# ArrowLuo/SegCLIP

Measured on AMD Instinct MI355X. Metric: image-text pairs/s fwd+bwd, ViT-B/16 224^2, per-GPU batch 256 (global 2048 at 8 GPUs), higher is better.
Workload: dtype bf16; 1 GPU; BASELINE configs[1]/[2]: ViT-B/16 224^2 + 77-token text, contrastive loss only; per_gpu_batch=256, global_batch=256, parallelism=dp1, attention_forward=bf16, residual_stream=fp32, cross_mode=t18, text_positions=all 77 (full context, as the reference computes it)

## Files before the change

### segclip_amd/csrc/attention.hip

```cpp
#include <stdlib.h>
#include <algorithm>
#include <atomic>

#include "common.h"

int segclip_gemm_f32_launch(const segclip_gemm_desc* d, hipStream_t stream);

namespace {

typedef __attribute__((address_space(3))) s16x4 lds_s16x4;

constexpr int ROWB = 128;

__device__ __forceinline__ int swz(int row, int col) {
  const int t = (row >> 1) & 7;
  const int f = ((t & 1) << 2) | (t >> 1);
  return row * ROWB + ((((col >> 3) ^ f)) << 4) + ((col & 7) << 1);
}

__device__ __forceinline__ bf16x8_t frag_rows(const char* t, int rbase, int kc, int lane) {
  return *reinterpret_cast<const bf16x8_t*>(t + swz(rbase + (lane & 31), kc * 16 + 8 * (lane >> 5)));
}
__device__ __forceinline__ bf16x8_t frag_tr(const char* t, int rbase, int cbase, int lane) {
  const int g4 = lane >> 4, q = lane & 15;
// ... 445 lines not shown
  stage_rows(Vt, Vp, a.v_st, 0, a.Tk, tkp, a.hd, tid, blockDim.x);
  __syncthreads();

  for (int q0 = wave * 32; q0 < tqp; q0 += nw * 32) {
    bf16x8_t qf[4], gf[4];
#pragma unroll
    for (int kc = 0; kc < 4; ++kc) {
      qf[kc] = frag_rows_g(Qp, a.q_st, q0, a.Tq, kc, lane, a.hd);
      gf[kc] = frag_rows_g(Gp, a.do_st, q0, a.Tq, kc, lane, a.hd);
    }
    const int q = q0 + li;
    const float lq = Ls[q], dq_ = Ds[q];
    f32x16 dq[2];
#pragma unroll
    for (int r = 0; r < 16; ++r) { dq[0][r] = 0.f; dq[1][r] = 0.f; }
    for (int k0 = 0; k0 < tkp; k0 += 32) {
      if (a.causal && k0 > q0 + 31) break;
      f32x16 s, dp;
#pragma unroll
      for (int r = 0; r < 16; ++r) { s[r] = 0.f; dp[r] = 0.f; }
#pragma unroll
      for (int kc = 0; kc < 4; ++kc) {
        s = __builtin_amdgcn_mfma_f32_32x32x16_bf16(frag_rows(Kt, k0, kc, lane), qf[kc], s, 0, 0, 0);
        dp = __builtin_amdgcn_mfma_f32_32x32x16_bf16(frag_rows(Vt, k0, kc, lane), gf[kc], dp, 0, 0, 0);
      }
      const bool edge = k0 + 32 > kvalid || q0 + 32 > a.Tq || (a.causal && k0 + 31 > q0);
      float ds[16];
      if (edge) {
#pragma unroll
        for (int r = 0; r < 16; ++r) {
          const int key = k0 + accrow(r, lh);
          const bool ok = key < kvalid && q < a.Tq && (!a.causal || key <= q);
          ds[r] = ok ? __builtin_amdgcn_exp2f(s[r] * sc2 - lq) * (dp[r] - dq_) : 0.f;
        }
      } else {
#pragma unroll
        for (int r = 0; r < 16; ++r) ds[r] = __builtin_amdgcn_exp2f(s[r] * sc2 - lq) * (dp[r] - dq_);
      }
      const bf16x8_t sb0 = pack8(ds), sb1 = pack8(ds + 8);
#pragma unroll
      for (int dt = 0; dt < 2; ++dt) {
        dq[dt] = __builtin_amdgcn_mfma_f32_32x32x16_bf16(frag_tr(Kt, k0, dt * 32, lane), sb0, dq[dt], 0, 0, 0);
        dq[dt] = __builtin_amdgcn_mfma_f32_32x32x16_bf16(frag_tr(Kt, k0 + 16, dt * 32, lane), sb1, dq[dt], 0, 0, 0);
      }
    }
#pragma unroll
    for (int r = 0; r < 16; ++r) { dq[0][r] *= a.scale; dq[1][r] *= a.scale; }
    store_acc_T(a.dQ + b * a.dq_sb + hoff, a.dq_st, q, a.Tq, a.hd, dq, lh);
  }

  if (a.colsum_part) {
    const int c = tid & 7, nrl = (int)blockDim.x >> 3;
    float accq[8];
#pragma unroll
    for (int j = 0; j < 8; ++j) accq[j] = 0.f;
    for (int r = tid >> 3; r < tkp; r += nrl) {
      const u32x4 kv = *reinterpret_cast<const u32x4*>(Kt + swz(r, c * 8));
      const float w = Cs[r];
#pragma unroll
      for (int j = 0; j < 4; ++j) {
        accq[2 * j] += w * __uint_as_float(kv[j] << 16);
        accq[2 * j + 1] += w * __uint_as_float(kv[j] & 0xffff0000u);
      }
    }
#pragma unroll
    for (int j = 0; j < 8; ++j) {
      float vq = accq[j], vv = accv[j];
      vq += __shfl_xor(vq, 8, 64); vv += __shfl_xor(vv, 8, 64);
      vq += __shfl_xor(vq, 16, 64); vv += __shfl_xor(vv, 16, 64);
      vq += __shfl_xor(vq, 32, 64); vv += __shfl_xor(vv, 32, 64);
      if (lane < 8) {
        Red[(wave * 3 + 0) * 64 + c * 8 + j] = vq;
        Red[(wave * 3 + 2) * 64 + c * 8 + j] = vv;
      }
    }
    __syncthreads();
    for (int t = tid; t < 192; t += (int)blockDim.x) {
      const int m = t >> 6, dd = t & 63;
      float v = 0.f;
      if (m != 1)
        for (int w = 0; w < nw; ++w) v += Red[(w * 3 + m) * 64 + dd];
      if (dd < a.hd) a.colsum_part[((int64_t)b * 3 + m) * ((int64_t)a.H * a.hd) + hoff + dd] = v;
    }
  }
}

#include "attention_sp.inc"
#include "attention_pf.inc"
#include "attention_spl.inc"
#include "attention_dqw.inc"
#include "attention_stream.inc"

__global__ void softmax_rows_kernel(float* __restrict__ S, int64_t rows, int Tq, int Tk, int causal, const int* klen,
                                    int H) {
  const int lane = threadIdx.x & 63;
  const int64_t row = (int64_t)blockIdx.x * (blockDim.x >> 6) + (threadIdx.x >> 6);
  if (row >= rows) return;
  const int q = (int)(row % Tq);
  float* s = S + row * Tk;
  int lim = causal ? (q + 1 < Tk ? q + 1 : Tk) : Tk;
  if (klen) { const int kv = klen[row / ((int64_t)H * Tq)]; lim = kv < lim ? kv : lim; }
  float mx = -INFINITY;
  for (int c = lane; c < lim; c += 64) mx = fmaxf(mx, s[c]);
  mx = wave_max(mx);
  float sum = 0.f;
  for (int c = lane; c < lim; c += 64) sum += expf(s[c] - mx);
  sum = wave_sum(sum);
  const float inv = 1.f / sum;
  for (int c = lane; c < Tk; c += 64) s[c] = c < lim ? expf(s[c] - mx) * inv : 0.f;
}
__global__ void softmax_bwd_rows_kernel(const float* __restrict__ P, float* __restrict__ dP, int64_t rows, int Tk,
                                        float scale) {
  const int lane = threadIdx.x & 63;
  const int64_t row = (int64_t)blockIdx.x * (blockDim.x >> 6) + (threadIdx.x >> 6);
  if (row >= rows) return;
  const float* p = P + row * Tk;
  float* d = dP + row * Tk;
  float dot = 0.f;
  for (int c = lane; c < Tk; c += 64) dot += p[c] * d[c];
  dot = wave_sum(dot);
  for (int c = lane; c < Tk; c += 64) d[c] = p[c] * (d[c] - dot) * scale;
}


bool bf16_ok(const segclip_attn_desc* d) {
  const int64_t s[] = {d->q_sb, d->q_st, d->k_sb, d->k_st, d->v_sb, d->v_st, d->o_sb, d->o_st};
  for (int64_t v : s) if (v % 8) return false;
  return d->hd % 8 == 0 && d->hd <= 64;
}

struct Tuning {
  int smallq = segclip_tuning_int("SEGCLIP_ATTN_SMALLQ", 1);
  int fwd_staged = segclip_tuning_int("SEGCLIP_ATTN_FWD_STAGED", -1), fwd_lean = segclip_tuning_int("SEGCLIP_ATTN_FWD_LEAN", 1);
  int fwd_pf = segclip_tuning_int("SEGCLIP_ATTN_FWD_PF", 1), fwd_grid = segclip_tuning_int("SEGCLIP_ATTN_FWD_GRID", 0);
  int bwd_dqw_long = segclip_tuning_int("SEGCLIP_ATTN_BWD_DQW_LONG", 1), bwd_dqw = segclip_tuning_int("SEGCLIP_ATTN_BWD_DQW", 1);
  int bwd_sp = segclip_tuning_int("SEGCLIP_ATTN_BWD_SP", 1), bwd_spl = segclip_tuning_int("SEGCLIP_ATTN_BWD_SPL", 1);
  int bwd_grid = segclip_tuning_int("SEGCLIP_ATTN_BWD_GRID", -1), bwd_waves = segclip_tuning_int("SEGCLIP_ATTN_BWD_WAVES", 0);
};
const Tuning& tuning() { static const Tuning t; return t; }

struct Plan {
  int route, tiles, variant;
  int waves;
  size_t lds;
  int staged;
};
int tiles_of(const segclip_attn_desc* d) { return (int)cdiv(d->Tq > d->Tk ? d->Tq : d->Tk, 32); }
bool long_seq(const segclip_attn_desc* d) { return d->Tq > TMAX || d->Tk > TMAX; }

Plan plan_fwd(const segclip_attn_desc* d) {
  const Tuning& t = tuning();
  if (d->dtype != SEGCLIP_BF16) return {SEGCLIP_ATTN_ROUTE_F32, tiles_of(d)};
  const int staged = t.fwd_staged >= 0 ? t.fwd_staged : (d->Tq > 128 ? 1 : 0);
  if (t.smallq && smallq::covers(d)) return {SEGCLIP_ATTN_ROUTE_SMALLQ, 1, 0, smallq::WPB_FWD, smallq::lds_bytes((int)d->Tk, false), staged};
  const int tiles = (int)cdiv(d->Tq, 32);
  const size_t pf_lds = fwd_pf_lds_bytes(tiles, (int)d->Tq);
  if (t.fwd_pf && d->Tq == d->Tk && !(d->flags & SEGCLIP_ATTN_FP8) && (tiles == 3 || tiles == 6 || tiles == 7) && pf_lds <= 160 * 1024)
    return {SEGCLIP_ATTN_ROUTE_PF, tiles, d->causal ? 1 : 0, tiles + 1, pf_lds, staged};
  const int nw = tiles < 8 ? tiles : (tiles <= 8 ? 8 : (int)cdiv(tiles, cdiv(tiles, 8)));
  return {SEGCLIP_ATTN_ROUTE_GENERIC, tiles, (staged ? 1 : 0) | nw << 8, nw, 0, staged};
}

Plan plan_bwd(const segclip_attn_desc* d) {
  const Tuning& t = tuning();
  const int tiles = tiles_of(d);
  if (d->dtype != SEGCLIP_BF16) return {SEGCLIP_ATTN_ROUTE_F32, tiles};
  if (t.smallq && smallq::covers(d)) return {SEGCLIP_ATTN_ROUTE_SMALLQ, 1, 0, smallq::WPB_BWD, smallq::lds_bytes((int)d->Tk, true)};
  if (long_seq(d)) {
    if (t.bwd_dqw_long && d->Tq == d->Tk && !d->causal && d->hd == 64 && d->Tq % 32 <= 30 && d->Tq % 224 != 0)
      return {SEGCLIP_ATTN_ROUTE_DQW, 7, 1, 8, bwd_dqw_lds_bytes<7>()};
    return {SEGCLIP_ATTN_ROUTE_STREAM, tiles, 0, 0, bwd_stream_lds_bytes()};
  }
  const bool masked = d->causal || d->klen;
  if (t.bwd_sp && d->Tq == d->Tk) {
    if (t.bwd_dqw && !masked && d->hd == 64 && tiles == 7 && d->Tq % 32 >= 1 && d->Tq % 32 <= 30)
      return {SEGCLIP_ATTN_ROUTE_DQW, 7, 0, 8, bwd_dqw_lds_bytes<7>()};
    const size_t spl_lds = bwd_spl_lds_bytes((int)d->Tq);
    if (t.bwd_spl && !masked && d->hd == 64 && tiles >= 5 && tiles <= 7 && spl_lds <= 160 * 1024)
      return {SEGCLIP_ATTN_ROUTE_SPL, tiles, 0, tiles + 1, spl_lds};
    return {SEGCLIP_ATTN_ROUTE_SP, tiles, masked ? 1 : 0, tiles, bwd_sp_lds_bytes(tiles * 32)};
  }
  int nw = tiles < 4 ? tiles : 4;
  if (t.bwd_waves >= 1 && t.bwd_waves <= 8) nw = tiles < t.bwd_waves ? tiles : t.bwd_waves;
  return {SEGCLIP_ATTN_ROUTE_TWOPASS, tiles, nw << 8, nw, bwd_lds_bytes(tiles * 32)};
}

constexpr int MAX_DEVICES = 64;
struct Device { int index, ncu; };
std::atomic<int> device_ncu[MAX_DEVICES];
std::atomic<int> pf_per_cu[MAX_DEVICES][2][8][33];

bool current_device(Device& dv) {
  if (hipGetDevice(&dv.index) != hipSuccess || dv.index < 0 || dv.index >= MAX_DEVICES) return false;
  if ((dv.ncu = device_ncu[dv.index]) == 0) {
    if (hipDeviceGetAttribute(&dv.ncu, hipDeviceAttributeMultiprocessorCount, dv.index) != hipSuccess || dv.ncu <= 0) dv.ncu = 256;
    device_ncu[dv.index] = dv.ncu;
  }
  return true;
}

template <auto KERNEL>
int raise_lds_limit(const char* who, const Device& dv, size_t bytes) {
  static std::atomic<bool> done[MAX_DEVICES];
  if (done[dv.index]) return 0;
  const hipError_t e = hipFuncSetAttribute(reinterpret_cast<const void*>(KERNEL), hipFuncAttributeMaxDynamicSharedMemorySize, (int)bytes);
  SEGCLIP_REQUIRE(e == hipSuccess, "%s bf16: cannot raise the dynamic LDS limit: %s", who, hipGetErrorString(e));
  done[dv.index] = true;
  return 0;
}

template <auto KERNEL, typename... Args>
int launch(const char* name, dim3 grid, int waves, const Plan& p, hipStream_t stream, const Args&... args) {
  hipLaunchKernelGGL(KERNEL, grid, dim3(waves * 64), p.lds, stream, args...);
  SEGCLIP_CHECK_LAUNCH(name);
  return 0;
}

template <int NT, bool CAUSAL>
int launch_fwd_pf_as(const FwdArgs& a, const Plan& p, int nitems, hipStream_t stream) {
  Device dv;
  SEGCLIP_REQUIRE(current_device(dv), "attn_fwd: cannot query the current device");
  if (int rc = raise_lds_limit<attn_fwd_pf_kernel<NT, CAUSAL>>("attn_fwd", dv, 160 * 1024)) return rc;
  std::atomic<int>& cached = pf_per_cu[dv.index][CAUSAL][NT][pf_kv_rows(a.Tq) >> 3];
  int per_cu = cached;
  if (per_cu == 0) {
    if (hipOccupancyMaxActiveBlocksPerMultiprocessor(&per_cu, attn_fwd_pf_kernel<NT, CAUSAL>, p.waves * 64, p.lds) != hipSuccess || per_cu < 1) per_cu = 1;
    if (tuning().fwd_grid > 0) per_cu = tuning().fwd_grid;
    cached = per_cu;
  }
  return launch<attn_fwd_pf_kernel<NT, CAUSAL>>("attn_fwd_pf", dim3(std::min(nitems, dv.ncu * per_cu)), p.waves, p, stream, a, nitems);
}
int launch_fwd_pf(const FwdArgs& a, const Plan& p, int nitems, hipStream_t stream) {
  switch (p.tiles * 2 + p.variant) {
    case 3 * 2: return launch_fwd_pf_as<3, false>(a, p, nitems, stream);
    case 3 * 2 + 1: return launch_fwd_pf_as<3, true>(a, p, nitems, stream);
    case 6 * 2: return launch_fwd_pf_as<6, false>(a, p, nitems, stream);
    case 6 * 2 + 1: return launch_fwd_pf_as<6, true>(a, p, nitems, stream);
    case 7 * 2: return launch_fwd_pf_as<7, false>(a, p, nitems, stream);
    default: return launch_fwd_pf_as<7, true>(a, p, nitems, stream);
  }
}

int launch_fwd_generic(const segclip_attn_desc* d, const FwdArgs& a, const Plan& p, hipStream_t stream) {
  SEGCLIP_REQUIRE(d->B * d->H <= 65535, "attn_fwd: B*H too large");
  if (d->flags & SEGCLIP_ATTN_FP8) {
    segclip_set_error("attn_fwd: the e4m3 forward was removed (slower than bf16 at head_dim 64, DESIGN.md section 8): "
                      "configs[4] runs bf16 attention");
    return SEGCLIP_ERR_UNSUPPORTED;
  }
  return launch<attn_fwd_bf16_kernel>("attn_fwd_bf16", dim3((unsigned)cdiv(p.tiles, p.waves), (unsigned)(d->B * d->H)), p.waves, p, stream, a);
}

struct Mat { const void* p; int64_t s0, sk, sb, sh; };
int gemm_f32(const segclip_attn_desc* d, hipStream_t stream, int64_t M, int64_t N, int64_t K, Mat A, Mat B, Mat C, float alpha = 1.f) {
  segclip_gemm_desc g{};
  g.nb1 = d->B; g.nb2 = d->H;
  g.a_dtype = g.b_dtype = g.c_dtype = g.r_dtype = SEGCLIP_F32;
  g.alpha = alpha;
  g.A = A.p; g.B = B.p; g.C = const_cast<void*>(C.p); g.M = M; g.N = N; g.K = K;
  g.sam = A.s0; g.sak = A.sk; g.sbn = B.s0; g.sbk = B.sk; g.ldc = C.s0;
  g.bsA1 = A.sb; g.bsA2 = A.sh; g.bsB1 = B.sb; g.bsB2 = B.sh; g.bsC1 = C.sb; g.bsC2 = C.sh;
  return segclip_gemm_f32_launch(&g, stream);
}
Mat scores(const segclip_attn_desc* d, const void* p, bool transposed) {
  return transposed ? Mat{p, 1, d->Tk, d->H * d->Tq * d->Tk, d->Tq * d->Tk} : Mat{p, d->Tk, 1, d->H * d->Tq * d->Tk, d->Tq * d->Tk};
}

int launch_fwd_f32(const segclip_attn_desc* d, hipStream_t stream) {
  float* P = (float*)d->stats;
  if (int rc = gemm_f32(d, stream, d->Tq, d->Tk, d->hd, {d->Q, d->q_st, 1, d->q_sb, d->hd}, {d->K, d->k_st, 1, d->k_sb, d->hd}, scores(d, P, false), d->scale)) return rc;
  const int64_t rows = d->B * d->H * d->Tq;
  hipLaunchKernelGGL(softmax_rows_kernel, dim3((unsigned)cdiv(rows, 4)), dim3(256), 0, stream, P, rows, (int)d->Tq,
                     (int)d->Tk, d->causal, (const int*)d->klen, (int)d->H);
  SEGCLIP_CHECK_LAUNCH("attn_softmax_rows");
  return gemm_f32(d, stream, d->Tq, d->hd, d->Tk, scores(d, P, false), {d->V, 1, d->v_st, d->v_sb, d->hd}, {d->O, d->o_st, 1, d->o_sb, d->hd});
}

template <bool MULTI>
int launch_bwd_dqw(const BwdArgs& a, const Plan& p, const Device& dv, hipStream_t stream) {
  if (int rc = raise_lds_limit<attn_bwd_dqw_bf16_kernel<7, MULTI>>("attn_bwd", dv, 160 * 1024)) return rc;
  return launch<attn_bwd_dqw_bf16_kernel<7, MULTI>>("attn_bwd_dqw_bf16", dim3(std::min(a.nitems, dv.ncu)), p.waves, p, stream, a);
}

int launch_bwd_stream(const segclip_attn_desc* d, const BwdArgs& a, const Plan& p, const Device& dv, hipStream_t stream) {
  if (raise_lds_limit<attn_bwd_dkv_stream_kernel>("attn_bwd", dv, p.lds) || raise_lds_limit<attn_bwd_dq_stream_kernel>("attn_bwd", dv, p.lds))
    SEGCLIP_REQUIRE(false, "attn_bwd bf16: cannot raise the dynamic LDS limit");
  const int ktiles = (int)cdiv(d->Tk, 32), qtiles = (int)cdiv(d->Tq, 32);
  const int nwk = ktiles < 8 ? ktiles : 8, nwq = qtiles < 8 ? qtiles : 8;
  if (int rc = launch<attn_bwd_dkv_stream_kernel>("attn_bwd_dkv_stream", dim3(a.nitems, (unsigned)cdiv(ktiles, nwk)), nwk, p, stream, a, a.ws)) return rc;
  return launch<attn_bwd_dq_stream_kernel>("attn_bwd_dq_stream", dim3(a.nitems, (unsigned)cdiv(qtiles, nwq)), nwq, p, stream, a, (const float*)a.ws);
}

dim3 bwd_persistent_grid(int nitems, const Device& dv, int per_cu) {
  const int env = tuning().bwd_grid;
  return dim3((unsigned)(env == 0 ? nitems : std::min<int64_t>(nitems, (int64_t)dv.ncu * (env > 0 ? env : per_cu))));
}
int launch_bwd_spl(const BwdArgs& a, const Plan& p, const Device& dv, hipStream_t stream) {
  if (int rc = raise_lds_limit<attn_bwd_spl_bf16_kernel>("attn_bwd", dv, 160 * 1024)) return rc;
  return launch<attn_bwd_spl_bf16_kernel>("attn_bwd_spl_bf16", bwd_persistent_grid(a.nitems, dv, 1), p.waves, p, stream, a);
}
template <bool MASKED>
int launch_bwd_sp(const BwdArgs& a, const Plan& p, const Device& dv, hipStream_t stream) {
  if (int rc = raise_lds_limit<attn_bwd_sp_bf16_kernel<MASKED>>("attn_bwd", dv, bwd_sp_lds_bytes(TMAX))) return rc;
  int per_cu = 0;
  if (hipOccupancyMaxActiveBlocksPerMultiprocessor(&per_cu, attn_bwd_sp_bf16_kernel<MASKED>, p.waves * 64, p.lds) != hipSuccess || per_cu < 1) per_cu = 1;
  return launch<attn_bwd_sp_bf16_kernel<MASKED>>("attn_bwd_sp_bf16", bwd_persistent_grid(a.nitems, dv, per_cu), p.waves, p, stream, a);
}

int launch_bwd_twopass(const BwdArgs& a, const Plan& p, const Device& dv, hipStream_t stream) {
  if (int rc = raise_lds_limit<attn_bwd_bf16_kernel>("attn_bwd", dv, bwd_lds_bytes(TMAX))) return rc;
  return launch<attn_bwd_bf16_kernel>("attn_bwd_bf16", dim3(a.nitems), p.waves, p, stream, a);
}

int launch_bwd_f32(const segclip_attn_desc* d, hipStream_t stream) {
  SEGCLIP_REQUIRE(d->colsum_part == nullptr, "attn_bwd f32: colsum_part is a bf16-path feature");
  SEGCLIP_REQUIRE(d->ws != nullptr, "attn_bwd f32: workspace required");
  const float* P = (const float*)d->stats;
  float* dP = (float*)d->ws;
  const Mat dO = {d->dO, d->do_st, 1, d->do_sb, d->hd}, dO_T = {d->dO, 1, d->do_st, d->do_sb, d->hd};
  int rc;
// ... 110 lines not shown
```

### segclip_amd/csrc/attention_smallq.inc

```
namespace smallq {

constexpr int QMAX = 8, WPB_FWD = 4, WPB_BWD = 2;

static inline size_t lds_bytes(int S, bool bwd) {
  return (size_t)(bwd ? WPB_BWD : WPB_FWD) * ((bwd ? 2 : 1) * QMAX * 64 + (bwd ? 2 : 1) * (size_t)S * QMAX) * sizeof(float);
}

__device__ __forceinline__ void unpack8f(const u32x4 v, float* f) {
#pragma unroll
  for (int j = 0; j < 4; ++j) { f[2 * j] = __uint_as_float(v[j] << 16); f[2 * j + 1] = __uint_as_float(v[j] & 0xffff0000u); }
}
__device__ __forceinline__ void stage_q(float* dst, const bf16_t* base, int64_t st, int nq, int lane) {
  const int r = lane >> 3, c = lane & 7;
  float f[8];
  if (r < nq) unpack8f(*reinterpret_cast<const u32x4*>(base + (int64_t)r * st + c * 8), f);
  else {
#pragma unroll
    for (int j = 0; j < 8; ++j) f[j] = 0.f;
  }
  *reinterpret_cast<f32x4*>(dst + r * 64 + c * 8) = f32x4{f[0], f[1], f[2], f[3]};
  *reinterpret_cast<f32x4*>(dst + r * 64 + c * 8 + 4) = f32x4{f[4], f[5], f[6], f[7]};
}
__device__ __forceinline__ void row_dots(const bf16_t* row, const float* qs, float (&s)[QMAX]) {
  v2f acc[QMAX];
#pragma unroll
  for (int q = 0; q < QMAX; ++q) acc[q] = v2f{0.f, 0.f};
#pragma unroll
  for (int c = 0; c < 8; ++c) {
    float kf[8];
    unpack8f(*reinterpret_cast<const u32x4*>(row + c * 8), kf);
    const v2f k0 = v2f{kf[0], kf[1]}, k1 = v2f{kf[2], kf[3]}, k2 = v2f{kf[4], kf[5]}, k3 = v2f{kf[6], kf[7]};
#pragma unroll
    for (int q = 0; q < QMAX; ++q) {
      const f32x4 a = *reinterpret_cast<const f32x4*>(qs + q * 64 + c * 8), b = *reinterpret_cast<const f32x4*>(qs + q * 64 + c * 8 + 4);
      acc[q] += k0 * v2f{a[0], a[1]};
      acc[q] += k1 * v2f{a[2], a[3]};
      acc[q] += k2 * v2f{b[0], b[1]};
      acc[q] += k3 * v2f{b[2], b[3]};
    }
  }
#pragma unroll
  for (int q = 0; q < QMAX; ++q) s[q] = acc[q][0] + acc[q][1];
}

__global__ __launch_bounds__(WPB_FWD * 64) void attn_smallq_fwd_kernel(FwdArgs a, int nitems) {
  extern __shared__ float smq[];
  const int lane = threadIdx.x & 63, wave = threadIdx.x >> 6;
  const int item = blockIdx.x * WPB_FWD + wave;
  if (item >= nitems) return;
  const int b = item / a.H, h = item % a.H, S = a.Tk, nq = a.Tq;
  float* qs = smq + (size_t)wave * (QMAX * 64 + (size_t)S * QMAX);
  float* ps = qs + QMAX * 64;
  const bf16_t* Qp = a.Q + (int64_t)b * a.q_sb + (int64_t)h * 64;
  const bf16_t* Kp = a.K + (int64_t)b * a.k_sb + (int64_t)h * 64;
  const bf16_t* Vp = a.V + (int64_t)b * a.v_sb + (int64_t)h * 64;
  stage_q(qs, Qp, a.q_st, nq, lane);
  __builtin_amdgcn_wave_barrier();
  float mx[QMAX];
#pragma unroll
  for (int q = 0; q < QMAX; ++q) mx[q] = -INFINITY;
  for (int key = lane; key < S; key += 64) {
    float s[QMAX];
    row_dots(Kp + (int64_t)key * a.k_st, qs, s);
#pragma unroll
    for (int q = 0; q < QMAX; ++q) { s[q] *= a.scale; mx[q] = fmaxf(mx[q], s[q]); }
    *reinterpret_cast<f32x4*>(ps + (size_t)key * QMAX) = f32x4{s[0], s[1], s[2], s[3]};
    *reinterpret_cast<f32x4*>(ps + (size_t)key * QMAX + 4) = f32x4{s[4], s[5], s[6], s[7]};
  }
  float sum[QMAX];
#pragma unroll
  for (int q = 0; q < QMAX; ++q) { mx[q] = wave_max(mx[q]); sum[q] = 0.f; }
  for (int key = lane; key < S; key += 64) {
    float* p = ps + (size_t)key * QMAX;
#pragma unroll
    for (int q = 0; q < QMAX; ++q) { const float e = __expf(p[q] - mx[q]); p[q] = e; sum[q] += e; }
  }
  float inv[QMAX];
#pragma unroll
  for (int q = 0; q < QMAX; ++q) {
    sum[q] = wave_sum(sum[q]);
    inv[q] = 1.f / sum[q];
    if (lane == q && q < nq) a.lse[((int64_t)b * a.H + h) * nq + q] = mx[q] + __logf(sum[q]);
  }
  __builtin_amdgcn_wave_barrier();
  v2f o2[QMAX / 2];
#pragma unroll
  for (int q = 0; q < QMAX / 2; ++q) o2[q] = v2f{0.f, 0.f};
  const bf16_t* vcol = Vp + lane;
  int key = 0;
#define SMQ_FWD_BATCH(U)                                                                                                  \
  for (; key + U <= S; key += U) {                                                                                        \
    float v[U];                                                                                                           \
    _Pragma("unroll") for (int u = 0; u < U; ++u) v[u] = bf2f(vcol[(int64_t)(key + u) * a.v_st]);                       \
    _Pragma("unroll") for (int u = 0; u < U; ++u) {                                                                      \
      const f32x4 p0 = *reinterpret_cast<const f32x4*>(ps + (size_t)(key + u) * QMAX),                                    \
                  p1 = *reinterpret_cast<const f32x4*>(ps + (size_t)(key + u) * QMAX + 4);                                \
      const v2f vv = v2f{v[u], v[u]};                                                                                     \
      o2[0] += v2f{p0[0], p0[1]} * vv; o2[1] += v2f{p0[2], p0[3]} * vv;                                                   \
      o2[2] += v2f{p1[0], p1[1]} * vv; o2[3] += v2f{p1[2], p1[3]} * vv;                                                   \
    }                                                                                                                     \
  }
  SMQ_FWD_BATCH(4)
#undef SMQ_FWD_BATCH
  for (; key < S; ++key) {
    const float v = bf2f(vcol[(int64_t)key * a.v_st]);
    const float* p = ps + (size_t)key * QMAX;
    const v2f vv = v2f{v, v};
#pragma unroll
    for (int q = 0; q < QMAX / 2; ++q) o2[q] += v2f{p[2 * q], p[2 * q + 1]} * vv;
  }
  bf16_t* Op = a.O + (int64_t)b * a.o_sb + (int64_t)h * 64 + lane;
#pragma unroll
  for (int q = 0; q < QMAX; ++q)
    if (q < nq) Op[(int64_t)q * a.o_st] = f2bf(o2[q >> 1][q & 1] * inv[q]);
}

__global__ __launch_bounds__(WPB_BWD * 64) void attn_smallq_bwd_kernel(BwdArgs a, int nitems) {
  extern __shared__ float smq[];
  const int lane = threadIdx.x & 63, wave = threadIdx.x >> 6;
  const int item = blockIdx.x * WPB_BWD + wave;
  if (item >= nitems) return;
  const int b = item / a.H, h = item % a.H, S = a.Tk, nq = a.Tq;
  float* qs = smq + (size_t)wave * (2 * QMAX * 64 + 2 * (size_t)S * QMAX);
  float* dos = qs + QMAX * 64;
  float* ps = dos + QMAX * 64;
  float* dss = ps + (size_t)S * QMAX;
  const bf16_t* Qp = a.Q + (int64_t)b * a.q_sb + (int64_t)h * 64;
  const bf16_t* Kp = a.K + (int64_t)b * a.k_sb + (int64_t)h * 64;
  const bf16_t* Vp = a.V + (int64_t)b * a.v_sb + (int64_t)h * 64;
  const bf16_t* Op = a.O + (int64_t)b * a.o_sb + (int64_t)h * 64;
  const bf16_t* dOp = a.dO + (int64_t)b * a.do_sb + (int64_t)h * 64;
  stage_q(qs, Qp, a.q_st, nq, lane);
  stage_q(dos, dOp, a.do_st, nq, lane);
  float dd[QMAX], lse[QMAX];
#pragma unroll
  for (int q = 0; q < QMAX; ++q) {
    const float ov = q < nq ? bf2f(Op[(int64_t)q * a.o_st + lane]) : 0.f, gv = q < nq ? bf2f(dOp[(int64_t)q * a.do_st + lane]) : 0.f;
    dd[q] = wave_sum(ov * gv);
    lse[q] = q < nq ? a.lse[((int64_t)b * a.H + h) * nq + q] : INFINITY;
  }
  __builtin_amdgcn_wave_barrier();
  for (int key = lane; key < S; key += 64) {
    float s[QMAX], dp[QMAX];
    row_dots(Kp + (int64_t)key * a.k_st, qs, s);
    row_dots(Vp + (int64_t)key * a.v_st, dos, dp);
    float p[QMAX], ds[QMAX];
#pragma unroll
    for (int q = 0; q < QMAX; ++q) { p[q] = __expf(s[q] * a.scale - lse[q]); ds[q] = p[q] * (dp[q] - dd[q]) * a.scale; }
    *reinterpret_cast<f32x4*>(ps + (size_t)key * QMAX) = f32x4{p[0], p[1], p[2], p[3]};
    *reinterpret_cast<f32x4*>(ps + (size_t)key * QMAX + 4) = f32x4{p[4], p[5], p[6], p[7]};
    *reinterpret_cast<f32x4*>(dss + (size_t)key * QMAX) = f32x4{ds[0], ds[1], ds[2], ds[3]};
    *reinterpret_cast<f32x4*>(dss + (size_t)key * QMAX + 4) = f32x4{ds[4], ds[5], ds[6], ds[7]};
  }
  __builtin_amdgcn_wave_barrier();
  float qd[QMAX], god[QMAX];
  v2f dq2[QMAX / 2], qd2[QMAX / 2], god2[QMAX / 2];
#pragma unroll
  for (int q = 0; q < QMAX; ++q) { qd[q] = qs[q * 64 + lane]; god[q] = dos[q * 64 + lane]; }
#pragma unroll
  for (int q = 0; q < QMAX / 2; ++q) { dq2[q] = v2f{0.f, 0.f}; qd2[q] = v2f{qd[2 * q], qd[2 * q + 1]}; god2[q] = v2f{god[2 * q], god[2 * q + 1]}; }
  const bf16_t* kcol = Kp + lane;
  bf16_t* dKp = a.dK + (int64_t)b * a.dk_sb + (int64_t)h * 64 + lane;
  bf16_t* dVp = a.dV + (int64_t)b * a.dv_sb + (int64_t)h * 64 + lane;
  int key = 0;
#define SMQ_BWD_BATCH(U)                                                                                                  \
  for (; key + U <= S; key += U) {                                                                                        \
    float kv[U];                                                                                                          \
    _Pragma("unroll") for (int u = 0; u < U; ++u) kv[u] = bf2f(kcol[(int64_t)(key + u) * a.k_st]);                      \
    _Pragma("unroll") for (int u = 0; u < U; ++u) {                                                                      \
      const float* p = ps + (size_t)(key + u) * QMAX;                                                                     \
      const float* ds = dss + (size_t)(key + u) * QMAX;                                                                   \
      const f32x4 p0 = *reinterpret_cast<const f32x4*>(p), p1 = *reinterpret_cast<const f32x4*>(p + 4);                  \
      const f32x4 s0 = *reinterpret_cast<const f32x4*>(ds), s1 = *reinterpret_cast<const f32x4*>(ds + 4);                \
      const v2f pa = v2f{p0[0], p0[1]}, pb = v2f{p0[2], p0[3]}, pc = v2f{p1[0], p1[1]}, pd = v2f{p1[2], p1[3]};           \
      const v2f sa = v2f{s0[0], s0[1]}, sb = v2f{s0[2], s0[3]}, sc = v2f{s1[0], s1[1]}, sd = v2f{s1[2], s1[3]};           \
      const v2f dv2 = (pa * god2[0] + pb * god2[1]) + (pc * god2[2] + pd * god2[3]);                                      \
      const v2f dk2 = (sa * qd2[0] + sb * qd2[1]) + (sc * qd2[2] + sd * qd2[3]);                                          \
      dVp[(int64_t)(key + u) * a.dv_st] = f2bf(dv2[0] + dv2[1]);                                                          \
      dKp[(int64_t)(key + u) * a.dk_st] = f2bf(dk2[0] + dk2[1]);                                                          \
      const v2f kk = v2f{kv[u], kv[u]};                                                                                   \
      dq2[0] += sa * kk; dq2[1] += sb * kk; dq2[2] += sc * kk; dq2[3] += sd * kk;                                         \
    }                                                                                                                     \
  }
  SMQ_BWD_BATCH(16)
  SMQ_BWD_BATCH(4)
#undef SMQ_BWD_BATCH
  for (; key < S; ++key) {
    const float kv = bf2f(kcol[(int64_t)key * a.k_st]);
    const float* p = ps + (size_t)key * QMAX;
    const float* ds = dss + (size_t)key * QMAX;
    float dv = 0.f, dk = 0.f;
#pragma unroll
    for (int q = 0; q < QMAX; ++q) { dv += p[q] * god[q]; dk += ds[q] * qd[q]; dq2[q >> 1][q & 1] += ds[q] * kv; }
    dVp[(int64_t)key * a.dv_st] = f2bf(dv);
    dKp[(int64_t)key * a.dk_st] = f2bf(dk);
  }
  bf16_t* dQp = a.dQ + (int64_t)b * a.dq_sb + (int64_t)h * 64 + lane;
#pragma unroll
  for (int q = 0; q < QMAX; ++q)
    if (q < nq) dQp[(int64_t)q * a.dq_st] = f2bf(dq2[q >> 1][q & 1]);
  if (a.colsum_part) {
    float sq = 0.f, sv = 0.f;
#pragma unroll
    for (int q = 0; q < QMAX; ++q)
      if (q < nq) { sq += dq2[q >> 1][q & 1]; sv += god[q]; }
    float* cp = a.colsum_part + (int64_t)b * 3 * ((int64_t)a.H * 64) + (int64_t)h * 64 + lane;
    cp[0] = sq;
    cp[(int64_t)a.H * 64] = 0.f;
    cp[2 * (int64_t)a.H * 64] = sv;
  }
}

static inline bool covers(const segclip_attn_desc* d) {
  return d->dtype == SEGCLIP_BF16 && d->hd == 64 && d->Tq >= 1 && d->Tq <= QMAX && d->Tk >= 1 && !d->causal && d->klen == nullptr &&
         !(d->flags & SEGCLIP_ATTN_FP8) && lds_bytes((int)d->Tk, true) <= 64 * 1024 && lds_bytes((int)d->Tk, false) <= 64 * 1024;
}

}
```

Measured before the change: 7327 pairs/s.

## Rewrite small-query attention kernels with MFMA scores and streamed key tiles

Replaces the scalar per-lane dot-product small-query attention forward and backward kernels with a tiled design. K/V are streamed in 32-key tiles through LDS with register prefetch of the next tile, scores are computed via bf16 MFMA 16x16x32, and the forward pass uses an online softmax. LDS per wave becomes fixed rather than proportional to Tk, and the backward pass uses 4 waves per block. dK/dV are staged back through LDS for coalesced writes. It also caps Tk at 448 for this route, so longer key lengths fall back to the other attention routes.

Result: no change. 7396 pairs/s (median of 6 runs) (+0.9%).

```diff
diff --git a/segclip_amd/csrc/attention.hip b/segclip_amd/csrc/attention.hip
--- a/segclip_amd/csrc/attention.hip
+++ b/segclip_amd/csrc/attention.hip
@@ -621,7 +621,7 @@
   const Tuning& t = tuning();
   if (d->dtype != SEGCLIP_BF16) return {SEGCLIP_ATTN_ROUTE_F32, tiles_of(d)};
   const int staged = t.fwd_staged >= 0 ? t.fwd_staged : (d->Tq > 128 ? 1 : 0);
-  if (t.smallq && smallq::covers(d)) return {SEGCLIP_ATTN_ROUTE_SMALLQ, 1, 0, smallq::WPB_FWD, smallq::lds_bytes((int)d->Tk, false), staged};
+  if (t.smallq && smallq::covers(d)) return {SEGCLIP_ATTN_ROUTE_SMALLQ, 1, 0, smallq::WPB, smallq::lds_bytes(false), staged};
   const int tiles = (int)cdiv(d->Tq, 32);
   const size_t pf_lds = fwd_pf_lds_bytes(tiles, (int)d->Tq);
   if (t.fwd_pf && d->Tq == d->Tk && !(d->flags & SEGCLIP_ATTN_FP8) && (tiles == 3 || tiles == 6 || tiles == 7) && pf_lds <= 160 * 1024)
@@ -634,7 +634,7 @@
   const Tuning& t = tuning();
   const int tiles = tiles_of(d);
   if (d->dtype != SEGCLIP_BF16) return {SEGCLIP_ATTN_ROUTE_F32, tiles};
-  if (t.smallq && smallq::covers(d)) return {SEGCLIP_ATTN_ROUTE_SMALLQ, 1, 0, smallq::WPB_BWD, smallq::lds_bytes((int)d->Tk, true)};
+  if (t.smallq && smallq::covers(d)) return {SEGCLIP_ATTN_ROUTE_SMALLQ, 1, 0, smallq::WPB, smallq::lds_bytes(true)};
   if (long_seq(d)) {
     if (t.bwd_dqw_long && d->Tq == d->Tk && !d->causal && d->hd == 64 && d->Tq % 32 <= 30 && d->Tq % 224 != 0)
       return {SEGCLIP_ATTN_ROUTE_DQW, 7, 1, 8, bwd_dqw_lds_bytes<7>()};
diff --git a/segclip_amd/csrc/attention_smallq.inc b/segclip_amd/csrc/attention_smallq.inc
--- a/segclip_amd/csrc/attention_smallq.inc
+++ b/segclip_amd/csrc/attention_smallq.inc
@@ -1,219 +1,270 @@
 namespace smallq {
 
-constexpr int QMAX = 8, WPB_FWD = 4, WPB_BWD = 2;
-
-static inline size_t lds_bytes(int S, bool bwd) {
-  return (size_t)(bwd ? WPB_BWD : WPB_FWD) * ((bwd ? 2 : 1) * QMAX * 64 + (bwd ? 2 : 1) * (size_t)S * QMAX) * sizeof(float);
-}
-
+constexpr int QMAX = 8, KT = 32, WPB = 4;
+constexpr int TK_MAX = 448;
+constexpr int ROWP = 144;
+constexpr int TILE_B = KT * ROWP;
+constexpr int WAVE_LDS_FWD = 2 * TILE_B + KT * QMAX * 4, WAVE_LDS_BWD = 2 * TILE_B + 2 * KT * QMAX * 4;
+
+static inline size_t lds_bytes(bool bwd) { return (size_t)WPB * (bwd ? WAVE_LDS_BWD : WAVE_LDS_FWD); }
+
+__device__ __forceinline__ void wave_sync() {
+  __builtin_amdgcn_fence(__ATOMIC_ACQ_REL, "wavefront");
+  __builtin_amdgcn_wave_barrier();
+}
+__device__ __forceinline__ v2f unpack2f(uint32_t w) { return v2f{__uint_as_float(w << 16), __uint_as_float(w & 0xffff0000u)}; }
 __device__ __forceinline__ void unpack8f(const u32x4 v, float* f) {
 #pragma unroll
   for (int j = 0; j < 4; ++j) { f[2 * j] = __uint_as_float(v[j] << 16); f[2 * j + 1] = __uint_as_float(v[j] & 0xffff0000u); }
 }
-__device__ __forceinline__ void stage_q(float* dst, const bf16_t* base, int64_t st, int nq, int lane) {
-  const int r = lane >> 3, c = lane & 7;
-  float f[8];
-  if (r < nq) unpack8f(*reinterpret_cast<const u32x4*>(base + (int64_t)r * st + c * 8), f);
-  else {
-#pragma unroll
-    for (int j = 0; j < 8; ++j) f[j] = 0.f;
-  }
-  *reinterpret_cast<f32x4*>(dst + r * 64 + c * 8) = f32x4{f[0], f[1], f[2], f[3]};
-  *reinterpret_cast<f32x4*>(dst + r * 64 + c * 8 + 4) = f32x4{f[4], f[5], f[6], f[7]};
-}
-__device__ __forceinline__ void row_dots(const bf16_t* row, const float* qs, float (&s)[QMAX]) {
-  v2f acc[QMAX];
-#pragma unroll
-  for (int q = 0; q < QMAX; ++q) acc[q] = v2f{0.f, 0.f};
-#pragma unroll
-  for (int c = 0; c < 8; ++c) {
-    float kf[8];
-    unpack8f(*reinterpret_cast<const u32x4*>(row + c * 8), kf);
-    const v2f k0 = v2f{kf[0], kf[1]}, k1 = v2f{kf[2], kf[3]}, k2 = v2f{kf[4], kf[5]}, k3 = v2f{kf[6], kf[7]};
-#pragma unroll
-    for (int q = 0; q < QMAX; ++q) {
-      const f32x4 a = *reinterpret_cast<const f32x4*>(qs + q * 64 + c * 8), b = *reinterpret_cast<const f32x4*>(qs + q * 64 + c * 8 + 4);
-      acc[q] += k0 * v2f{a[0], a[1]};
-      acc[q] += k1 * v2f{a[2], a[3]};
-      acc[q] += k2 * v2f{b[0], b[1]};
-      acc[q] += k3 * v2f{b[2], b[3]};
-    }
-  }
-#pragma unroll
-  for (int q = 0; q < QMAX; ++q) s[q] = acc[q][0] + acc[q][1];
-}
-
-__global__ __launch_bounds__(WPB_FWD * 64) void attn_smallq_fwd_kernel(FwdArgs a, int nitems) {
-  extern __shared__ float smq[];
-  const int lane = threadIdx.x & 63, wave = threadIdx.x >> 6;
-  const int item = blockIdx.x * WPB_FWD + wave;
+__device__ __forceinline__ float lane_value(float v, int l) { return __int_as_float(__builtin_amdgcn_readlane(__float_as_int(v), l)); }
+__device__ __forceinline__ float quad_sum(float v) { v += __shfl_xor(v, 16, 64); return v + __shfl_xor(v, 32, 64); }
+__device__ __forceinline__ float quad_max(float v) { v = fmaxf(v, __shfl_xor(v, 16, 64)); return fmaxf(v, __shfl_xor(v, 32, 64)); }
+
+struct TileRegs { u32x4 v[KT / 8]; };
+__device__ __forceinline__ void tile_load(TileRegs& r, const bf16_t* base, int64_t st, int key0, int S, int lane) {
+#pragma unroll
+  for (int i = 0; i < KT / 8; ++i) {
+    const int row = key0 + (lane >> 3) + 8 * i;
+    r.v[i] = *reinterpret_cast<const u32x4*>(base + (int64_t)(row < S ? row : S - 1) * st + (lane & 7) * 8);
+  }
+}
+__device__ __forceinline__ void tile_write(char* t, const TileRegs& r, int key0, int S, int lane) {
+#pragma unroll
+  for (int i = 0; i < KT / 8; ++i) {
+    const int row = (lane >> 3) + 8 * i;
+    *reinterpret_cast<u32x4*>(t + row * ROWP + (lane & 7) * 16) = key0 + row < S ? r.v[i] : u32x4{0u, 0u, 0u, 0u};
+  }
+}
+__device__ __forceinline__ void tile_store(bf16_t* base, int64_t st, const char* t, int key0, int S, int lane) {
+#pragma unroll
+  for (int i = 0; i < KT / 8; ++i) {
+    const int row = (lane >> 3) + 8 * i;
+    const u32x4 v = *reinterpret_cast<const u32x4*>(t + row * ROWP + (lane & 7) * 16);
+    if (key0 + row < S) *reinterpret_cast<u32x4*>(base + (int64_t)(key0 + row) * st + (lane & 7) * 8) = v;
+  }
+}
+__device__ __forceinline__ void query_frags(bf16x8_t (&f)[2], const bf16_t* base, int64_t st, int nq, int lane) {
+  const int q = lane & 15;
+#pragma unroll
+  for (int ks = 0; ks < 2; ++ks) {
+    const u32x4 raw = *reinterpret_cast<const u32x4*>(base + (int64_t)(q < nq ? q : nq - 1) * st + 32 * ks + 8 * (lane >> 4));
+    f[ks] = __builtin_bit_cast(bf16x8_t, q < nq ? raw : u32x4{0u, 0u, 0u, 0u});
+  }
+}
+__device__ __forceinline__ f32x4 score_block(const char* t, int rb, const bf16x8_t (&xf)[2], int lane) {
+  f32x4 acc = f32x4{0.f, 0.f, 0.f, 0.f};
+#pragma unroll
+  for (int ks = 0; ks < 2; ++ks) {
+    const bf16x8_t kf = *reinterpret_cast<const bf16x8_t*>(t + (16 * rb + (lane & 15)) * ROWP + 64 * ks + 16 * (lane >> 4));
+    acc = __builtin_amdgcn_mfma_f32_16x16x32_bf16(kf, xf[ks], acc, 0, 0, 0);
+  }
+  return acc;
+}
+__device__ __forceinline__ void rows_out(bf16_t* base, int64_t st, char* t, const v2f (&x)[QMAX], int nq, int lane) {
+  if (lane < 32) {
+#pragma unroll
+    for (int q = 0; q < QMAX; ++q) *reinterpret_cast<uint32_t*>(t + q * ROWP + 4 * lane) = pack2bf(x[q][0], x[q][1]);
+  }
+  wave_sync();
+  const u32x4 v = *reinterpret_cast<const u32x4*>(t + (lane >> 3) * ROWP + (lane & 7) * 16);
+  if ((lane >> 3) < nq) *reinterpret_cast<u32x4*>(base + (int64_t)(lane >> 3) * st + (lane & 7) * 8) = v;
+}
+
+__global__ __launch_bounds__(WPB * 64, 4) void attn_smallq_fwd_kernel(FwdArgs a, int nitems) {
+  extern __shared__ __attribute__((aligned(16))) char smq[];
+  const int lane = threadIdx.x & 63, wave = __builtin_amdgcn_readfirstlane(threadIdx.x >> 6);
+  const int item = blockIdx.x * WPB + wave;
   if (item >= nitems) return;
   const int b = item / a.H, h = item % a.H, S = a.Tk, nq = a.Tq;
-  float* qs = smq + (size_t)wave * (QMAX * 64 + (size_t)S * QMAX);
-  float* ps = qs + QMAX * 64;
-  const bf16_t* Qp = a.Q + (int64_t)b * a.q_sb + (int64_t)h * 64;
+  const int q16 = lane & 15, g = lane >> 4, half = lane >> 5, j32 = lane & 31;
+  char* Kt = smq + (size_t)wave * WAVE_LDS_FWD;
+  char* Vt = Kt + TILE_B;
+  float* ps = reinterpret_cast<float*>(Vt + TILE_B);
   const bf16_t* Kp = a.K + (int64_t)b * a.k_sb + (int64_t)h * 64;
   const bf16_t* Vp = a.V + (int64_t)b * a.v_sb + (int64_t)h * 64;
-  stage_q(qs, Qp, a.q_st, nq, lane);
-  __builtin_amdgcn_wave_barrier();
-  float mx[QMAX];
-#pragma unroll
-  for (int q = 0; q < QMAX; ++q) mx[q] = -INFINITY;
-  for (int key = lane; key < S; key += 64) {
-    float s[QMAX];
-    row_dots(Kp + (int64_t)key * a.k_st, qs, s);
-#pragma unroll
-    for (int q = 0; q < QMAX; ++q) { s[q] *= a.scale; mx[q] = fmaxf(mx[q], s[q]); }
-    *reinterpret_cast<f32x4*>(ps + (size_t)key * QMAX) = f32x4{s[0], s[1], s[2], s[3]};
-    *reinterpret_cast<f32x4*>(ps + (size_t)key * QMAX + 4) = f32x4{s[4], s[5], s[6], s[7]};
-  }
-  float sum[QMAX];
-#pragma unroll
-  for (int q = 0; q < QMAX; ++q) { mx[q] = wave_max(mx[q]); sum[q] = 0.f; }
-  for (int key = lane; key < S; key += 64) {
-    float* p = ps + (size_t)key * QMAX;
-#pragma unroll
-    for (int q = 0; q < QMAX; ++q) { const float e = __expf(p[q] - mx[q]); p[q] = e; sum[q] += e; }
-  }
-  float inv[QMAX];
+  TileRegs kr, vr;
+  tile_load(kr, Kp, a.k_st, 0, S, lane);
+  tile_load(vr, Vp, a.v_st, 0, S, lane);
+  bf16x8_t qf[2];
+  query_frags(qf, a.Q + (int64_t)b * a.q_sb + (int64_t)h * 64, a.q_st, nq, lane);
+  float m = -INFINITY, l = 0.f;
+  v2f o2[QMAX];
+#pragma unroll
+  for (int q = 0; q < QMAX; ++q) o2[q] = v2f{0.f, 0.f};
+  for (int key0 = 0; key0 < S; key0 += KT) {
+    tile_write(Kt, kr, key0, S, lane);
+    tile_write(Vt, vr, key0, S, lane);
+    if (key0 + KT < S) {
+      tile_load(kr, Kp, a.k_st, key0 + KT, S, lane);
+      tile_load(vr, Vp, a.v_st, key0 + KT, S, lane);
+    }
+    wave_sync();
+    float s[KT / 4];
+    float tmax = -INFINITY;
+#pragma unroll
+    for (int rb = 0; rb < KT / 16; ++rb) {
+      const f32x4 acc = score_block(Kt, rb, qf, lane);
+#pragma unroll
+      for (int r = 0; r < 4; ++r) {
+        s[4 * rb + r] = key0 + 16 * rb + 4 * g + r < S ? acc[r] * a.scale : -INFINITY;
+        tmax = fmaxf(tmax, s[4 * rb + r]);
+      }
+    }
+    tmax = quad_max(tmax);
+    const float mn = fmaxf(m, tmax);
+    const float alpha = __expf(m - mn);
+    float rs = 0.f;
+#pragma unroll
+    for (int rb = 0; rb < KT / 16; ++rb)
+#pragma unroll
+      for (int r = 0; r < 4; ++r) {
+        const float e = __expf(s[4 * rb + r] - mn);
+        rs += e;
+        if (q16 < QMAX) ps[(16 * rb + 4 * g + r) * QMAX + q16] = e;
+      }
+    l = l * alpha + quad_sum(rs);
+    m = mn;
+#pragma unroll
+    for (int q = 0; q < QMAX; ++q) {
+      const float aq = lane_value(alpha, q);
+      o2[q] *= v2f{aq, aq};
+    }
+    wave_sync();
+#pragma unroll 4
+    for (int kk = 0; kk < KT / 2; ++kk) {
+      const int key = 2 * kk + half;
+      const v2f vv = unpack2f(*reinterpret_cast<const uint32_t*>(Vt + key * ROWP + 4 * j32));
+      const f32x4 p0 = *reinterpret_cast<const f32x4*>(ps + key * QMAX), p1 = *reinterpret_cast<const f32x4*>(ps + key * QMAX + 4);
+      o2[0] += v2f{p0[0], p0[0]} * vv; o2[1] += v2f{p0[1], p0[1]} * vv; o2[2] += v2f{p0[2], p0[2]} * vv; o2[3] += v2f{p0[3], p0[3]} * vv;
+      o2[4] += v2f{p1[0], p1[0]} * vv; o2[5] += v2f{p1[1], p1[1]} * vv; o2[6] += v2f{p1[2], p1[2]} * vv; o2[7] += v2f{p1[3], p1[3]} * vv;
+    }
+    wave_sync();
+  }
+  const float inv = 1.f / l;
 #pragma unroll
   for (int q = 0; q < QMAX; ++q) {
-    sum[q] = wave_sum(sum[q]);
-    inv[q] = 1.f / sum[q];
-    if (lane == q && q < nq) a.lse[((int64_t)b * a.H + h) * nq + q] = mx[q] + __logf(sum[q]);
-  }
-  __builtin_amdgcn_wave_barrier();
-  v2f o2[QMAX / 2];
-#pragma unroll
-  for (int q = 0; q < QMAX / 2; ++q) o2[q] = v2f{0.f, 0.f};
-  const bf16_t* vcol = Vp + lane;
-  int key = 0;
-#define SMQ_FWD_BATCH(U)                                                                                                  \
-  for (; key + U <= S; key += U) {                                                                                        \
-    float v[U];                                                                                                           \
-    _Pragma("unroll") for (int u = 0; u < U; ++u) v[u] = bf2f(vcol[(int64_t)(key + u) * a.v_st]);                       \
-    _Pragma("unroll") for (int u = 0; u < U; ++u) {                                                                      \
-      const f32x4 p0 = *reinterpret_cast<const f32x4*>(ps + (size_t)(key + u) * QMAX),                                    \
-                  p1 = *reinterpret_cast<const f32x4*>(ps + (size_t)(key + u) * QMAX + 4);                                \
-      const v2f vv = v2f{v[u], v[u]};                                                                                     \
-      o2[0] += v2f{p0[0], p0[1]} * vv; o2[1] += v2f{p0[2], p0[3]} * vv;                                                   \
-      o2[2] += v2f{p1[0], p1[1]} * vv; o2[3] += v2f{p1[2], p1[3]} * vv;                                                   \
-    }                                                                                                                     \
-  }
-  SMQ_FWD_BATCH(4)
-#undef SMQ_FWD_BATCH
-  for (; key < S; ++key) {
-    const float v = bf2f(vcol[(int64_t)key * a.v_st]);
-    const float* p = ps + (size_t)key * QMAX;
-    const v2f vv = v2f{v, v};
-#pragma unroll
-    for (int q = 0; q < QMAX / 2; ++q) o2[q] += v2f{p[2 * q], p[2 * q + 1]} * vv;
-  }
-  bf16_t* Op = a.O + (int64_t)b * a.o_sb + (int64_t)h * 64 + lane;
-#pragma unroll
-  for (int q = 0; q < QMAX; ++q)
-    if (q < nq) Op[(int64_t)q * a.o_st] = f2bf(o2[q >> 1][q & 1] * inv[q]);
-}
-
-__global__ __launch_bounds__(WPB_BWD * 64) void attn_smallq_bwd_kernel(BwdArgs a, int nitems) {
-  extern __shared__ float smq[];
-  const int lane = threadIdx.x & 63, wave = threadIdx.x >> 6;
-  const int item = blockIdx.x * WPB_BWD + wave;
+    const float iq = lane_value(inv, q);
+    o2[q] = v2f{(o2[q][0] + __shfl_xor(o2[q][0], 32, 64)) * iq, (o2[q][1] + __shfl_xor(o2[q][1], 32, 64)) * iq};
+  }
+  rows_out(a.O + (int64_t)b * a.o_sb + (int64_t)h * 64, a.o_st, Kt, o2, nq, lane);
+  if (lane < nq) a.lse[((int64_t)b * a.H + h) * nq + lane] = m + __logf(l);
+}
+
+__global__ __launch_bounds__(WPB * 64, 3) void attn_smallq_bwd_kernel(BwdArgs a, int nitems) {
+  extern __shared__ __attribute__((aligned(16))) char smq[];
+  const int lane = threadIdx.x & 63, wave = __builtin_amdgcn_readfirstlane(threadIdx.x >> 6);
+  const int item = blockIdx.x * WPB + wave;
   if (item >= nitems) return;
   const int b = item / a.H, h = item % a.H, S = a.Tk, nq = a.Tq;
-  float* qs = smq + (size_t)wave * (2 * QMAX * 64 + 2 * (size_t)S * QMAX);
-  float* dos = qs + QMAX * 64;
-  float* ps = dos + QMAX * 64;
-  float* dss = ps + (size_t)S * QMAX;
+  const int q16 = lane & 15, g = lane >> 4, half = lane >> 5, j32 = lane & 31;
+  char* Kt = smq + (size_t)wave * WAVE_LDS_BWD;
+  char* Vt = Kt + TILE_B;
+  float* ps = reinterpret_cast<float*>(Vt + TILE_B);
+  float* dss = ps + KT * QMAX;
   const bf16_t* Qp = a.Q + (int64_t)b * a.q_sb + (int64_t)h * 64;
   const bf16_t* Kp = a.K + (int64_t)b * a.k_sb + (int64_t)h * 64;
   const bf16_t* Vp = a.V + (int64_t)b * a.v_sb + (int64_t)h * 64;
   const bf16_t* Op = a.O + (int64_t)b * a.o_sb + (int64_t)h * 64;
   const bf16_t* dOp = a.dO + (int64_t)b * a.do_sb + (int64_t)h * 64;
-  stage_q(qs, Qp, a.q_st, nq, lane);
-  stage_q(dos, dOp, a.do_st, nq, lane);
-  float dd[QMAX], lse[QMAX];
+  TileRegs kr, vr;
+  tile_load(kr, Kp, a.k_st, 0, S, lane);
+  tile_load(vr, Vp, a.v_st, 0, S, lane);
+  bf16x8_t qf[2], gf[2];
+  query_frags(qf, Qp, a.q_st, nq, lane);
+  query_frags(gf, dOp, a.do_st, nq, lane);
+  float dd, lse;
+  {
+    const int qc = q16 < nq ? q16 : nq - 1;
+    const u32x4* op = reinterpret_cast<const u32x4*>(Op + (int64_t)qc * a.o_st + 16 * g);
+    const u32x4* gp = reinterpret_cast<const u32x4*>(dOp + (int64_t)qc * a.do_st + 16 * g);
+    float of[16], gv[16];
+    unpack8f(op[0], of); unpack8f(op[1], of + 8);
+    unpack8f(gp[0], gv); unpack8f(gp[1], gv + 8);
+    float d = 0.f;
+#pragma unroll
+    for (int i = 0; i < 16; ++i) d += of[i] * gv[i];
+    d = quad_sum(d);
+    dd = q16 < nq ? d : 0.f;
+    const float ls = a.lse[((int64_t)b * a.H + h) * nq + qc];
+    lse = q16 < nq ? ls : INFINITY;
+  }
+  v2f qd2[QMAX], god2[QMAX], dq2[QMAX];
 #pragma unroll
   for (int q = 0; q < QMAX; ++q) {
-    const float ov = q < nq ? bf2f(Op[(int64_t)q * a.o_st + lane]) : 0.f, gv = q < nq ? bf2f(dOp[(int64_t)q * a.do_st + lane]) : 0.f;
-    dd[q] = wave_sum(ov * gv);
-    lse[q] = q < nq ? a.lse[((int64_t)b * a.H + h) * nq + q] : INFINITY;
-  }
-  __builtin_amdgcn_wave_barrier();
-  for (int key = lane; key < S; key += 64) {
-    float s[QMAX], dp[QMAX];
-    row_dots(Kp + (int64_t)key * a.k_st, qs, s);
-    row_dots(Vp + (int64_t)key * a.v_st, dos, dp);
-    float p[QMAX], ds[QMAX];
-#pragma unroll
-    for (int q = 0; q < QMAX; ++q) { p[q] = __expf(s[q] * a.scale - lse[q]); ds[q] = p[q] * (dp[q] - dd[q]) * a.scale; }
-    *reinterpret_cast<f32x4*>(ps + (size_t)key * QMAX) = f32x4{p[0], p[1], p[2], p[3]};
-    *reinterpret_cast<f32x4*>(ps + (size_t)key * QMAX + 4) = f32x4{p[4], p[5], p[6], p[7]};
-    *reinterpret_cast<f32x4*>(dss + (size_t)key * QMAX) = f32x4{ds[0], ds[1], ds[2], ds[3]};
-    *reinterpret_cast<f32x4*>(dss + (size_t)key * QMAX + 4) = f32x4{ds[4], ds[5], ds[6], ds[7]};
-  }
-  __builtin_amdgcn_wave_barrier();
-  float qd[QMAX], god[QMAX];
-  v2f dq2[QMAX / 2], qd2[QMAX / 2], god2[QMAX / 2];
-#pragma unroll
-  for (int q = 0; q < QMAX; ++q) { qd[q] = qs[q * 64 + lane]; god[q] = dos[q * 64 + lane]; }
-#pragma unroll
-  for (int q = 0; q < QMAX / 2; ++q) { dq2[q] = v2f{0.f, 0.f}; qd2[q] = v2f{qd[2 * q], qd[2 * q + 1]}; god2[q] = v2f{god[2 * q], god[2 * q + 1]}; }
-  const bf16_t* kcol = Kp + lane;
-  bf16_t* dKp = a.dK + (int64_t)b * a.dk_sb + (int64_t)h * 64 + lane;
-  bf16_t* dVp = a.dV + (int64_t)b * a.dv_sb + (int64_t)h * 64 + lane;
-  int key = 0;
-#define SMQ_BWD_BATCH(U)                                                                                                  \
-  for (; key + U <= S; key += U) {                                                                                        \
-    float kv[U];                                                                                                          \
-    _Pragma("unroll") for (int u = 0; u < U; ++u) kv[u] = bf2f(kcol[(int64_t)(key + u) * a.k_st]);                      \
-    _Pragma("unroll") for (int u = 0; u < U; ++u) {                                                                      \
-      const float* p = ps + (size_t)(key + u) * QMAX;                                                                     \
-      const float* ds = dss + (size_t)(key + u) * QMAX;                                                                   \
-      const f32x4 p0 = *reinterpret_cast<const f32x4*>(p), p1 = *reinterpret_cast<const f32x4*>(p + 4);                  \
-      const f32x4 s0 = *reinterpret_cast<const f32x4*>(ds), s1 = *reinterpret_cast<const f32x4*>(ds + 4);                \
-      const v2f pa = v2f{p0[0], p0[1]}, pb = v2f{p0[2], p0[3]}, pc = v2f{p1[0], p1[1]}, pd = v2f{p1[2], p1[3]};           \
-      const v2f sa = v2f{s0[0], s0[1]}, sb = v2f{s0[2], s0[3]}, sc = v2f{s1[0], s1[1]}, sd = v2f{s1[2], s1[3]};           \
-      const v2f dv2 = (pa * god2[0] + pb * god2[1]) + (pc * god2[2] + pd * god2[3]);                                      \
-      const v2f dk2 = (sa * qd2[0] + sb * qd2[1]) + (sc * qd2[2] + sd * qd2[3]);                                          \
-      dVp[(int64_t)(key + u) * a.dv_st] = f2bf(dv2[0] + dv2[1]);                                                          \
-      dKp[(int64_t)(key + u) * a.dk_st] = f2bf(dk2[0] + dk2[1]);                                                          \
-      const v2f kk = v2f{kv[u], kv[u]};                                                                                   \
-      dq2[0] += sa * kk; dq2[1] += sb * kk; dq2[2] += sc * kk; dq2[3] += sd * kk;                                         \
-    }                                                                                                                     \
-  }
-  SMQ_BWD_BATCH(16)
-  SMQ_BWD_BATCH(4)
-#undef SMQ_BWD_BATCH
-  for (; key < S; ++key) {
-    const float kv = bf2f(kcol[(int64_t)key * a.k_st]);
-    const float* p = ps + (size_t)key * QMAX;
-    const float* ds = dss + (size_t)key * QMAX;
-    float dv = 0.f, dk = 0.f;
-#pragma unroll
-    for (int q = 0; q < QMAX; ++q) { dv += p[q] * god[q]; dk += ds[q] * qd[q]; dq2[q >> 1][q & 1] += ds[q] * kv; }
-    dVp[(int64_t)key * a.dv_st] = f2bf(dv);
-    dKp[(int64_t)key * a.dk_st] = f2bf(dk);
-  }
-  bf16_t* dQp = a.dQ + (int64_t)b * a.dq_sb + (int64_t)h * 64 + lane;
+    dq2[q] = v2f{0.f, 0.f};
+    const int qc = q < nq ? q : nq - 1;
+    const uint32_t qw = *reinterpret_cast<const uint32_t*>(Qp + (int64_t)qc * a.q_st + 2 * j32);
+    const uint32_t gw = *reinterpret_cast<const uint32_t*>(dOp + (int64_t)qc * a.do_st + 2 * j32);
+    qd2[q] = unpack2f(q < nq ? qw : 0u);
+    god2[q] = unpack2f(q < nq ? gw : 0u);
+  }
+  bf16_t* dKp = a.dK + (int64_t)b * a.dk_sb + (int64_t)h * 64;
+  bf16_t* dVp = a.dV + (int64_t)b * a.dv_sb + (int64_t)h * 64;
+  for (int key0 = 0; key0 < S; key0 += KT) {
+    tile_write(Kt, kr, key0, S, lane);
+    tile_write(Vt, vr, key0, S, lane);
+    if (key0 + KT < S) {
+      tile_load(kr, Kp, a.k_st, key0 + KT, S, lane);
+      tile_load(vr, Vp, a.v_st, key0 + KT, S, lane);
+    }
+    wave_sync();
+#pragma unroll
+    for (int rb = 0; rb < KT / 16; ++rb) {
+      const f32x4 sa = score_block(Kt, rb, qf, lane), pa = score_block(Vt, rb, gf, lane);
+#pragma unroll
+      for (int r = 0; r < 4; ++r) {
+        const int kl = 16 * rb + 4 * g + r;
+        const float p = key0 + kl < S ? __expf(sa[r] * a.scale - lse) : 0.f;
+        const float ds = p * (pa[r] - dd) * a.scale;
+        if (q16 < QMAX) { ps[kl * QMAX + q16] = p; dss[kl * QMAX + q16] = ds; }
+      }
+    }
+    wave_sync();
+#pragma unroll 1
+    for (int kk = 0; kk < KT / 2; ++kk) {
+      const int key = 2 * kk + half;
+      uint32_t* kw = reinterpret_cast<uint32_t*>(Kt + key * ROWP + 4 * j32);
+      uint32_t* vw = reinterpret_cast<uint32_t*>(Vt + key * ROWP + 4 * j32);
+      const v2f kv = unpack2f(*kw);
+      const f32x4 p0 = *reinterpret_cast<const f32x4*>(ps + key * QMAX), p1 = *reinterpret_cast<const f32x4*>(ps + key * QMAX + 4);
+      const f32x4 s0 = *reinterpret_cast<const f32x4*>(dss + key * QMAX), s1 = *reinterpret_cast<const f32x4*>(dss + key * QMAX + 4);
+      const float p[QMAX] = {p0[0], p0[1], p0[2], p0[3], p1[0], p1[1], p1[2], p1[3]};
+      const float ds[QMAX] = {s0[0], s0[1], s0[2], s0[3], s1[0], s1[1], s1[2], s1[3]};
+      v2f dv = v2f{0.f, 0.f}, dk = v2f{0.f, 0.f};
+#pragma unroll
+      for (int q = 0; q < QMAX; ++q) {
+        dv += v2f{p[q], p[q]} * god2[q];
+        dk += v2f{ds[q], ds[q]} * qd2[q];
+        dq2[q] += v2f{ds[q], ds[q]} * kv;
+      }
+      *vw = pack2bf(dv[0], dv[1]);
+      *kw = pack2bf(dk[0], dk[1]);
+    }
+    wave_sync();
+    tile_store(dKp, a.dk_st, Kt, key0, S, lane);
+    tile_store(dVp, a.dv_st, Vt, key0, S, lane);
+    wave_sync();
+  }
 #pragma unroll
   for (int q = 0; q < QMAX; ++q)
-    if (q < nq) dQp[(int64_t)q * a.dq_st] = f2bf(dq2[q >> 1][q & 1]);
+    dq2[q] = v2f{dq2[q][0] + __shfl_xor(dq2[q][0], 32, 64), dq2[q][1] + __shfl_xor(dq2[q][1], 32, 64)};
+  rows_out(a.dQ + (int64_t)b * a.dq_sb + (int64_t)h * 64, a.dq_st, Kt, dq2, nq, lane);
   if (a.colsum_part) {
-    float sq = 0.f, sv = 0.f;
+    v2f sq = v2f{0.f, 0.f}, sv = v2f{0.f, 0.f};
 #pragma unroll
     for (int q = 0; q < QMAX; ++q)
-      if (q < nq) { sq += dq2[q >> 1][q & 1]; sv += god[q]; }
-    float* cp = a.colsum_part + (int64_t)b * 3 * ((int64_t)a.H * 64) + (int64_t)h * 64 + lane;
-    cp[0] = sq;
+      if (q < nq) { sq += dq2[q]; sv += god2[q]; }
+    float* cp = a.colsum_part + (int64_t)b * 3 * ((int64_t)a.H * 64) + (int64_t)h * 64 + 2 * j32 + half;
+    cp[0] = half ? sq[1] : sq[0];
     cp[(int64_t)a.H * 64] = 0.f;
-    cp[2 * (int64_t)a.H * 64] = sv;
+    cp[2 * (int64_t)a.H * 64] = half ? sv[1] : sv[0];
   }
 }
 
 static inline bool covers(const segclip_attn_desc* d) {
-  return d->dtype == SEGCLIP_BF16 && d->hd == 64 && d->Tq >= 1 && d->Tq <= QMAX && d->Tk >= 1 && !d->causal && d->klen == nullptr &&
-         !(d->flags & SEGCLIP_ATTN_FP8) && lds_bytes((int)d->Tk, true) <= 64 * 1024 && lds_bytes((int)d->Tk, false) <= 64 * 1024;
-}
-
-}
+  return d->dtype == SEGCLIP_BF16 && d->hd == 64 && d->Tq >= 1 && d->Tq <= QMAX && d->Tk >= 1 && d->Tk <= TK_MAX && !d->causal &&
+         d->klen == nullptr && !(d->flags & SEGCLIP_ATTN_FP8);
+}
+
+}
```
